# speedinghzl/DSRG

Hardware: AMD Instinct MI355X
Metric: images/sec DSRG train step (VGG16 321x321, 21-class) (higher is better)
Workload: dtype bf16 backbone (fp32 master weights) + f32/f64 supervision path

## Files before the change

dsrg_amd/csrc/conv_direct.hip:

```cpp
#include "common.h"

namespace dsrg {
namespace {
typedef __attribute__((ext_vector_type(8))) __bf16 bf16x8;
typedef __attribute__((ext_vector_type(2))) __bf16 bf16x2;
typedef __attribute__((ext_vector_type(2))) float f32x2;
typedef __attribute__((ext_vector_type(16))) float f32x16;
typedef __attribute__((address_space(3))) void lds_void;
constexpr int kTH = 8, kTW = 16;
constexpr int kHH = kTH + 2, kHW = kTW + 2;

template <int CIN, int COUT, int TPW_ = (CIN == 64 ? 2 : 1)> struct Cfg {
    static constexpr int CG = CIN / 16;
    static constexpr int KS = 9 * CG;
    static constexpr int TPW = TPW_;
    static constexpr int WGS = TPW * KS * 4 <= 144 ? 2 : 1;
    static constexpr int NG = COUT / (32 * TPW);
    static constexpr int PG = 4 / NG;
    static constexpr int MT = 4 / PG;
    static constexpr int KPS = WGS == 2 ? 2 : 4;
    static constexpr int SPT = CG / KPS;
    static constexpr int STEPS = 9 * SPT;
    static constexpr bool DMA = CIN == 128 && COUT == 128;
    static constexpr int CPR = CIN / 8;
    static constexpr int PB = (kHH * kHW + 63) / 64;
    static constexpr int PLANE = PB * 1024;
    static constexpr int NI = CPR * PB;
    static constexpr int IN_STRIDE = CIN * 2 + 16;
    static constexpr int OUT_STRIDE = COUT * 2 + 16;
    static constexpr int IN_BYTES = DMA && CPR * PLANE > kHH * kHW * IN_STRIDE ? CPR * PLANE : kHH * kHW * IN_STRIDE, OUT_BYTES = kTH * kTW * OUT_STRIDE;
    static constexpr int BUF = IN_BYTES > OUT_BYTES ? IN_BYTES : OUT_BYTES;
    static constexpr int VPP = CIN / 8;
    static constexpr int HALO_VECS = kHH * kHW * VPP;
    static constexpr int VPT = (HALO_VECS + 255) / 256;
    static constexpr int VPC = (VPT + MT - 1) / MT;
    static constexpr int OVP = COUT / 8;
    static constexpr int OVT = kTH * kTW * OVP / 256;
    static_assert(NG * PG == 4 && NG >= 1 && MT * PG == 4, "4 waves");
    static_assert(BUF % 16 == 0, "alignment");
};

struct ConvArgs {
    const uint16_t *x;
    const uint16_t *w;
    const float *bias;
    uint16_t *y;
    int B, H, W, relu, tiles_x, tiles_y, ntiles;
    const uint16_t *mask;
    float *colsum;
};

__device__ __forceinline__ uint32_t pack2(float lo, float hi) {
    f32x2 v = {lo, hi};
    bf16x2 b = __builtin_convertvector(v, bf16x2);
    return *reinterpret_cast<uint32_t *>(&b);
}

template <int CIN, int COUT, int TPW_, bool BWD = false>
__global__ __launch_bounds__(256, (TPW_ * CIN <= 64 ? 2 : 1)) void conv3x3_direct_kernel(ConvArgs a) {
    using C = Cfg<CIN, COUT, TPW_>;
    extern __shared__ __attribute__((aligned(16))) unsigned char conv_lds[];
    const int tid = threadIdx.x, lane = tid & 63, wave = tid >> 6;
    const int m = lane & 31, kgrp = lane >> 5;
    const int ng = wave % C::NG, pg = wave / C::NG;

    bf16x8 wf[C::TPW][C::KS];
#pragma unroll
    for (int j = 0; j < C::TPW; j++)
#pragma unroll
        for (int ks = 0; ks < C::KS; ks++)
            wf[j][ks] = *reinterpret_cast<const bf16x8 *>(a.w + (size_t)((ng * C::TPW + j) * 32 + m) * (9 * CIN) + ks * 16 + kgrp * 8);

    constexpr bool kBiasRegs = C::WGS == 1;
    float bias_r[kBiasRegs ? C::TPW : 1][4][4];
    if (kBiasRegs) {
#pragma unroll
        for (int j = 0; j < C::TPW; j++)
#pragma unroll
            for (int q = 0; q < 4; q++)
#pragma unroll
                for (int e = 0; e < 4; e++)
                    bias_r[j][q][e] = a.bias ? a.bias[(ng * C::TPW + j) * 32 + q * 8 + kgrp * 4 + e] : 0.0f;
    }

    auto tile_origin = [&](int t, int &b, int &y0, int &x0) {
        const int per = a.tiles_x * a.tiles_y;
        b = t / per;
        const int r = t - b * per;
        y0 = (r / a.tiles_x) * kTH;
        x0 = (r % a.tiles_x) * kTW;
    };
    constexpr bool kDma = C::DMA && !BWD;
    const rsrc_t rxh = make_rsrc(a.x, (size_t)a.B * a.H * a.W * CIN * 2);
    auto issue_halo = [&](int t, unsigned char *buf) {
        int b, y0, x0;
        tile_origin(t, b, y0, x0);
        const int wv = __builtin_amdgcn_readfirstlane(wave);
        uint32_t poff[C::PB];
#pragma unroll
        for (int blk = 0; blk < C::PB; blk++) {
            const int px = blk * 64 + lane, hy = px / kHW, hx = px - hy * kHW, yy = y0 - 1 + hy, xx = x0 - 1 + hx;
            const bool in = px < kHH * kHW && yy >= 0 && yy < a.H && xx >= 0 && xx < a.W;
            poff[blk] = in ? (uint32_t)((b * a.H + yy) * a.W + xx) * (uint32_t)(CIN * 2) : 0x80000000u;
        }
#pragma unroll
        for (int u = 0; u < (C::NI + 3) / 4; u++) {
            const int q = wv + 4 * u;
            if (q < C::NI) {
                const int c = q / C::PB, blk = q - c * C::PB;
                uint32_t off = poff[0];
#pragma unroll
                for (int k = 1; k < C::PB; k++) off = blk == k ? poff[k] : off;
                __builtin_amdgcn_raw_ptr_buffer_load_lds(rxh, (lds_void *)(buf + q * 1024), 16, off, (uint32_t)(c * 16), 0, 0);
            }
        }
    };
    uint4 pre[C::VPC];
    auto fetch = [&](int t, int c) {
        int b, y0, x0;
        tile_origin(t, b, y0, x0);
#pragma unroll
        for (int u = 0; u < C::VPC; u++) {
            const int v = tid + (c * C::VPC + u) * 256;
            uint4 val = make_uint4(0u, 0u, 0u, 0u);
            if (v < C::HALO_VECS) {
                const int px = v / C::VPP, cg = v % C::VPP, hy = px / kHW, hx = px - hy * kHW;
                const int yy = y0 - 1 + hy, xx = x0 - 1 + hx;
                if (yy >= 0 && yy < a.H && xx >= 0 && xx < a.W)
                    val = *reinterpret_cast<const uint4 *>(a.x + (((size_t)b * a.H + yy) * a.W + xx) * CIN + cg * 8);
            }
            pre[u] = val;
        }
    };
    auto park = [&](unsigned char *buf, int c) {
#pragma unroll
        for (int u = 0; u < C::VPC; u++) {
            const int v = tid + (c * C::VPC + u) * 256;
            if (v < C::HALO_VECS) *reinterpret_cast<uint4 *>(buf + (v / C::VPP) * C::IN_STRIDE + (v % C::VPP) * 16) = pre[u];
        }
    };

    int t = blockIdx.x, cur = 0;
    if (t >= a.ntiles) return;
    if constexpr (kDma) {
        issue_halo(t, conv_lds);
        asm volatile("s_waitcnt vmcnt(0)" ::: "memory");
    } else {
#pragma unroll
        for (int c = 0; c < C::MT; c++) {
            fetch(t, c);
            park(conv_lds, c);
        }
    }
    __syncthreads();
    float *csl = reinterpret_cast<float *>(conv_lds + 2 * C::BUF) + tid * 8;
    if (BWD) {
#pragma unroll
        for (int e = 0; e < 8; e++) csl[e] = 0.0f;
    }
    unsigned char *mtile = conv_lds + 2 * C::BUF + 256 * 8 * sizeof(float);
    const rsrc_t rmask = make_rsrc(a.mask, BWD ? (size_t)a.B * a.H * a.W * COUT * 2 : 0);
    for (; t < a.ntiles; t += gridDim.x) {
        const int tn = t + gridDim.x;
        const bool more = tn < a.ntiles;
        unsigned char *in = conv_lds + cur * C::BUF, *other = conv_lds + (cur ^ 1) * C::BUF;
        if (BWD) {
            int b, y0, x0;
            tile_origin(t, b, y0, x0);
            const int wv = __builtin_amdgcn_readfirstlane(wave);
#pragma unroll
            for (int u = 0; u < C::OVT; u++) {
                const int v = tid + u * 256, px = v / C::OVP, cg = v % C::OVP;
                const int yy = y0 + (px >> 4), xx = x0 + (px & 15);
                const uint32_t off = (yy < a.H && xx < a.W) ? (uint32_t)((b * a.H + yy) * a.W + xx) * (uint32_t)(COUT * 2) + (uint32_t)(cg * 16) : 0x80000000u;
                __builtin_amdgcn_raw_ptr_buffer_load_lds(rmask, (lds_void *)(mtile + (u * 256 + wv * 64) * 16), 16, off, 0, 0, 0);
            }
        }
        if constexpr (kDma)
            if (more) issue_halo(tn, other);
        f32x16 acc[C::MT][C::TPW];
#pragma unroll
        for (int mt = 0; mt < C::MT; mt++) {
            if constexpr (!kDma)
                if (more) fetch(tn, mt);
#pragma unroll
            for (int j = 0; j < C::TPW; j++)
#pragma unroll
                for (int r = 0; r < 16; r++) acc[mt][j][r] = 0.0f;
            const int ty = 2 * (pg * C::MT + mt) + (m >> 4), tx = m & 15;
            const unsigned char *lane_base = kDma ? in + (ty * kHW + tx) * 16 + kgrp * C::PLANE : in + (ty * kHW + tx) * C::IN_STRIDE + kgrp * 16;
            auto a_ptr = [&](int s) {
                const int tap = s / C::SPT, h = s % C::SPT;
                return lane_base + ((tap / 3) * kHW + tap % 3) * (kDma ? 16 : C::IN_STRIDE) + h * (kDma ? 2 * C::KPS * C::PLANE : 32 * C::KPS);
            };
            constexpr int kFragStep = kDma ? 2 * C::PLANE : 32;
            bf16x8 ar[2][C::KPS];
#pragma unroll
            for (int i = 0; i < C::KPS; i++) ar[0][i] = *reinterpret_cast<const bf16x8 *>(a_ptr(0) + i * kFragStep);
#pragma unroll
            for (int s = 0; s < C::STEPS; s++) {
                if (s + 1 < C::STEPS) {
#pragma unroll
                    for (int i = 0; i < C::KPS; i++) ar[(s + 1) & 1][i] = *reinterpret_cast<const bf16x8 *>(a_ptr(s + 1) + i * kFragStep);
                }
                __builtin_amdgcn_sched_barrier(0);
#pragma unroll
                for (int i = 0; i < C::KPS; i++)
#pragma unroll
                    for (int j = 0; j < C::TPW; j++)
                        acc[mt][j] = __builtin_amdgcn_mfma_f32_32x32x16_bf16(wf[j][s * C::KPS + i], ar[s & 1][i], acc[mt][j], 0, 0, 0);
                __builtin_amdgcn_sched_barrier(0);
            }
            if constexpr (!kDma)
                if (more) park(other, mt);
        }
        __syncthreads();
        unsigned char *ot = in;
#pragma unroll
        for (int mt = 0; mt < C::MT; mt++) {
#pragma unroll
            for (int j = 0; j < C::TPW; j++) {
#pragma unroll
                for (int q = 0; q < 4; q++) {
                    const int c0 = (ng * C::TPW + j) * 32 + q * 8 + kgrp * 4;
                    float v[4], bq[4] = {0.0f, 0.0f, 0.0f, 0.0f};
                    if (!kBiasRegs && a.bias) {
                        const float4 b4 = *reinterpret_cast<const float4 *>(a.bias + c0);
                        bq[0] = b4.x; bq[1] = b4.y; bq[2] = b4.z; bq[3] = b4.w;
                    }
#pragma unroll
                    for (int e = 0; e < 4; e++) {
                        v[e] = acc[mt][j][q * 4 + e] + (kBiasRegs ? bias_r[j][q][e] : bq[e]);
                        if (a.relu) v[e] = fmaxf(v[e], 0.0f);
                    }
                    *reinterpret_cast<uint2 *>(ot + ((pg * C::MT + mt) * 32 + m) * C::OUT_STRIDE + c0 * 2) =
                        make_uint2(pack2(v[0], v[1]), pack2(v[2], v[3]));
                }
            }
        }
        if (BWD) asm volatile("s_waitcnt vmcnt(0)" ::: "memory");
        __syncthreads();
        {
            int b, y0, x0;
            tile_origin(t, b, y0, x0);
            float cs[8] = {0.f, 0.f, 0.f, 0.f, 0.f, 0.f, 0.f, 0.f};
#pragma unroll
            for (int u = 0; u < C::OVT; u++) {
                const int v = tid + u * 256, px = v / C::OVP, cg = v % C::OVP;
                const int yy = y0 + (px >> 4), xx = x0 + (px & 15);
                uint4 val = *reinterpret_cast<const uint4 *>(ot + px * C::OUT_STRIDE + cg * 16);
                if (BWD) {
                    uint32_t w4[4] = {val.x, val.y, val.z, val.w};
                    const uint4 mkv = *reinterpret_cast<const uint4 *>(mtile + v * 16);
                    const uint32_t y4[4] = {mkv.x, mkv.y, mkv.z, mkv.w};
#pragma unroll
                    for (int e = 0; e < 4; e++) {
                        w4[e] &= ((int16_t)(y4[e] & 0xffffu) > 0 ? 0x0000ffffu : 0u) | ((int32_t)y4[e] >= 0x10000 ? 0xffff0000u : 0u);
                        cs[2 * e] += __uint_as_float(w4[e] << 16);
                        cs[2 * e + 1] += __uint_as_float(w4[e] & 0xffff0000u);
                    }
                    val = make_uint4(w4[0], w4[1], w4[2], w4[3]);
                }
                if (yy < a.H && xx < a.W)
                    *reinterpret_cast<uint4 *>(a.y + (((size_t)b * a.H + yy) * a.W + xx) * COUT + cg * 8) = val;
            }
            if (BWD) {
#pragma unroll
                for (int e = 0; e < 8; e++) csl[e] += cs[e];
            }
        }
        if constexpr (kDma) asm volatile("s_waitcnt vmcnt(0)" ::: "memory");
        __syncthreads();
        cur ^= 1;
    }
    if (BWD) {
        const float *red = reinterpret_cast<const float *>(conv_lds + 2 * C::BUF);
        __syncthreads();
        if (tid < COUT) {
            const int cg = tid >> 3, e = tid & 7;
            float s0 = 0.0f, s1 = 0.0f;
#pragma unroll 4
            for (int i = 0; i < 256 / C::OVP; i += 2) {
                s0 += red[(cg + C::OVP * i) * 8 + e];
                s1 += red[(cg + C::OVP * (i + 1)) * 8 + e];
            }
            a.colsum[(size_t)blockIdx.x * COUT + tid] = s0 + s1;
        }
    }
}

template <int CIN, int COUT, int TPW_>
int variant_grid(const ConvArgs &a, int n_cus) {
    const int slots = n_cus * Cfg<CIN, COUT, TPW_>::WGS;
    return a.ntiles < slots ? a.ntiles : slots;
}
template <int CIN, int COUT, int TPW_, bool BWD>
int launch_variant(const ConvArgs &a, int n_cus, hipStream_t stream, int &grid) {
    using C = Cfg<CIN, COUT, TPW_>;
    static LdsGrant grant;
    if (C::DMA && !BWD && (size_t)a.B * a.H * a.W * CIN * 2 >= ((size_t)1 << 31)) return DSRG_ERR_UNSUPPORTED;
    grid = variant_grid<CIN, COUT, TPW_>(a, n_cus);
    const size_t lds = 2 * (size_t)C::BUF + (BWD ? 256 * 8 * sizeof(float) + (size_t)kTH * kTW * COUT * 2 : 0);
    if (int rc = ensure_dynamic_lds(reinterpret_cast<const void *>(&conv3x3_direct_kernel<CIN, COUT, TPW_, BWD>), lds, grant)) return rc;
    hipLaunchKernelGGL((conv3x3_direct_kernel<CIN, COUT, TPW_, BWD>), dim3(grid), dim3(256), lds, stream, a);
    DSRG_LAUNCH_CHECK();
    return DSRG_OK;
}
template <int CIN, int COUT, int TPW_>
int launch_shape(const ConvArgs &a, int n_cus, hipStream_t stream, int &grid) {
    return a.mask ? launch_variant<CIN, COUT, TPW_, true>(a, n_cus, stream, grid) : launch_variant<CIN, COUT, TPW_, false>(a, n_cus, stream, grid);
}
constexpr int kC3Pix = 8;

__global__ __launch_bounds__(256) void conv3x3_c3_kernel(ConvArgs a) {
    __shared__ __attribute__((aligned(16))) unsigned char halo[2][kHH * kHW * kC3Pix];
    __shared__ __attribute__((aligned(16))) unsigned char ot[kTH * kTW * 144];
    constexpr int kOutStride = 144;
    const int tid = threadIdx.x, lane = tid & 63, wave = tid >> 6;
    const int m = lane & 31, kgrp = lane >> 5;

    bf16x8 wf[2][3];
#pragma unroll
    for (int nt = 0; nt < 2; nt++)
#pragma unroll
        for (int s3 = 0; s3 < 3; s3++) {
            uint16_t v[8];
#pragma unroll
            for (int e = 0; e < 8; e++) {
                const int tap = 4 * s3 + 2 * kgrp + (e >> 2), c = e & 3;
                v[e] = (tap < 9 && c < 3) ? a.w[((nt * 32 + m) * 9 + tap) * 3 + c] : (uint16_t)0;
            }
            uint4 pk = make_uint4(v[0] | (uint32_t)v[1] << 16, v[2] | (uint32_t)v[3] << 16, v[4] | (uint32_t)v[5] << 16,
                                  v[6] | (uint32_t)v[7] << 16);
            wf[nt][s3] = *reinterpret_cast<bf16x8 *>(&pk);
        }
    float bias_r[2][4][4];
#pragma unroll
    for (int nt = 0; nt < 2; nt++)
#pragma unroll
        for (int q = 0; q < 4; q++)
#pragma unroll
            for (int e = 0; e < 4; e++) bias_r[nt][q][e] = a.bias ? a.bias[nt * 32 + q * 8 + kgrp * 4 + e] : 0.0f;
    int toff[3][2];
#pragma unroll
    for (int s3 = 0; s3 < 3; s3++)
#pragma unroll
        for (int h = 0; h < 2; h++) {
            const int tap = min(4 * s3 + 2 * kgrp + h, 8);
            toff[s3][h] = ((tap / 3) * kHW + tap % 3) * kC3Pix;
        }

    auto tile_origin = [&](int t, int &b, int &y0, int &x0) {
        const int per = a.tiles_x * a.tiles_y;
        b = t / per;
        const int r = t - b * per;
        y0 = (r / a.tiles_x) * kTH;
        x0 = (r % a.tiles_x) * kTW;
    };
    uint2 pre = make_uint2(0u, 0u);
    auto fetch = [&](int t) {
        int b, y0, x0;
        tile_origin(t, b, y0, x0);
        pre = make_uint2(0u, 0u);
        if (tid < kHH * kHW) {
            const int hy = tid / kHW, hx = tid - hy * kHW, yy = y0 - 1 + hy, xx = x0 - 1 + hx;
            if (yy >= 0 && yy < a.H && xx >= 0 && xx < a.W) {
                const uint16_t *p = a.x + (((size_t)b * a.H + yy) * a.W + xx) * 3;
                pre = make_uint2(p[0] | (uint32_t)p[1] << 16, p[2]);
            }
        }
    };
    auto park = [&](unsigned char *buf) {
        if (tid < kHH * kHW) *reinterpret_cast<uint2 *>(buf + tid * kC3Pix) = pre;
    };

    int t = blockIdx.x, cur = 0;
    if (t >= a.ntiles) return;
    fetch(t);
    park(halo[0]);
    __syncthreads();
    const int ty = 2 * wave + (m >> 4), tx = m & 15;
    const int pix_off = (ty * kHW + tx) * kC3Pix;
    for (; t < a.ntiles; t += gridDim.x) {
        const int tn = t + gridDim.x;
        const bool more = tn < a.ntiles;
        if (more) fetch(tn);
        const unsigned char *in = halo[cur] + pix_off;
        f32x16 acc0, acc1;
#pragma unroll
        for (int r = 0; r < 16; r++) { acc0[r] = 0.0f; acc1[r] = 0.0f; }
#pragma unroll
        for (int s3 = 0; s3 < 3; s3++) {
            const uint2 lo = *reinterpret_cast<const uint2 *>(in + toff[s3][0]), hi = *reinterpret_cast<const uint2 *>(in + toff[s3][1]);
            uint4 pk = make_uint4(lo.x, lo.y, hi.x, hi.y);
            const bf16x8 ar = *reinterpret_cast<bf16x8 *>(&pk);
            acc0 = __builtin_amdgcn_mfma_f32_32x32x16_bf16(wf[0][s3], ar, acc0, 0, 0, 0);
            acc1 = __builtin_amdgcn_mfma_f32_32x32x16_bf16(wf[1][s3], ar, acc1, 0, 0, 0);
        }
#pragma unroll
        for (int nt = 0; nt < 2; nt++) {
#pragma unroll
            for (int q = 0; q < 4; q++) {
                const int c0 = nt * 32 + q * 8 + kgrp * 4;
                float v[4];
#pragma unroll
                for (int e = 0; e < 4; e++) {
                    v[e] = (nt ? acc1[q * 4 + e] : acc0[q * 4 + e]) + bias_r[nt][q][e];
                    if (a.relu) v[e] = fmaxf(v[e], 0.0f);
                }
                *reinterpret_cast<uint2 *>(ot + (wave * 32 + m) * kOutStride + c0 * 2) = make_uint2(pack2(v[0], v[1]), pack2(v[2], v[3]));
            }
        }
        if (more) park(halo[cur ^ 1]);
        __syncthreads();
        {
            int b, y0, x0;
            tile_origin(t, b, y0, x0);
#pragma unroll
            for (int u = 0; u < 4; u++) {
                const int v = tid + u * 256, px = v >> 3, cg = v & 7;
                const int yy = y0 + (px >> 4), xx = x0 + (px & 15);
                if (yy < a.H && xx < a.W)
                    *reinterpret_cast<uint4 *>(a.y + (((size_t)b * a.H + yy) * a.W + xx) * 64 + cg * 8) =
                        *reinterpret_cast<const uint4 *>(ot + px * kOutStride + cg * 16);
            }
        }
        __syncthreads();
        cur ^= 1;
    }
}

typedef __attribute__((__vector_size__(4 * sizeof(__bf16)))) __bf16 bf16x4v;
#define DSRG_LDS __attribute__((address_space(3)))

template <int CO_TILES> struct WCfg {
    static constexpr int COUT = 32 * CO_TILES;
    static constexpr int THREADS = CO_TILES * 128;
    static constexpr int NT = 9;
    static constexpr int SX = 192;
    static constexpr int SG = COUT * 2 + 64;
    static constexpr int X_BYTES = kHH * kHW * SX, G_BYTES = kTH * kTW * SG, BUF = X_BYTES + G_BYTES;
    static constexpr int XV = kHH * kHW * 8, XVT = (XV + THREADS - 1) / THREADS;
    static constexpr int GVP = COUT / 8, GVT = kTH * kTW * GVP / THREADS;
    static constexpr int PART = COUT * 9 * 64;
    static constexpr int WGS = CO_TILES == 2 ? 2 : 1, NBUF = WGS == 2 ? 1 : 2;
};

struct WgradArgs {
    const uint16_t *x;
    const uint16_t *g;
    float *part;
    int B, H, W, cin, tiles_x, tiles_y, nitems, roles;
};

__device__ __forceinline__ bf16x8 tr_frag(DSRG_LDS unsigned char *p, int stride4) {
    bf16x4v lo = __builtin_amdgcn_ds_read_tr16_b64_v4bf16(reinterpret_cast<DSRG_LDS bf16x4v *>(p));
    bf16x4v hi = __builtin_amdgcn_ds_read_tr16_b64_v4bf16(reinterpret_cast<DSRG_LDS bf16x4v *>(p + stride4));
    return __builtin_shufflevector(lo, hi, 0, 1, 2, 3, 4, 5, 6, 7);
}

template <int CO_TILES>
__global__ __launch_bounds__(CO_TILES * 128, (CO_TILES == 2 ? 2 : 1)) void conv3x3_wgrad_kernel(WgradArgs a) {
    using C = WCfg<CO_TILES>;
// ... 202 lines not shown
#pragma unroll
    for (int r = 0; r < 16; r++) acc[r] = 0.0f;
    int t = blockIdx.x, cur = 0;
    if (t < a.nitems) {
        fetch(t);
        park(0);
    }
    __syncthreads();
    const int cpx = tid >> 1, chalf = tid & 1;
    const int cty = cpx >> 4, ctx_ = cpx & 15;
    for (; t < a.nitems; t += gridDim.x) {
        const int tn = t + gridDim.x;
        const bool more = tn < a.nitems;
        if (more) fetch(tn);
#pragma unroll
        for (int k = 0; k < 5; k++) {
            const int tap = chalf * 5 + k;
            if (tap < 9)
                *reinterpret_cast<uint2 *>(xc + cpx * kC3Row + tap * 8) =
                    *reinterpret_cast<const uint2 *>(halo(cur) + ((cty + tap / 3) * kHW + ctx_ + tap % 3) * kC3Pix);
        }
        __syncthreads();
        DSRG_LDS unsigned char *gb = (DSRG_LDS unsigned char *)gt(cur) + g_lane, *xb = (DSRG_LDS unsigned char *)xc + x_lane;
#pragma unroll
        for (int ks = 0; ks < kTH; ks++) {
            const bf16x8 ga = tr_frag(gb + ks * kTW * kC3Row, 4 * kC3Row), bx = tr_frag(xb + ks * kTW * kC3Row, 4 * kC3Row);
            acc = __builtin_amdgcn_mfma_f32_32x32x16_bf16(ga, bx, acc, 0, 0, 0);
        }
        if (more) park(cur ^ 1);
        __syncthreads();
        cur ^= 1;
    }
    float *pp = a.part + (size_t)blockIdx.x * 64 * 64;
#pragma unroll
    for (int r = 0; r < 16; r++) {
        const int o = otile * 32 + (r & 3) + 8 * (r >> 2) + 4 * (lane >> 5);
        pp[o * 64 + ntile * 32 + (lane & 31)] = acc[r];
    }
}

template <bool F32_OUT>
__global__ __launch_bounds__(1024) void conv3x3_c3_wgrad_reduce_kernel(const float *part, void *gw, int nwg) {
    __shared__ float red[kRedChunks][64];
    const int el = threadIdx.x & 63, ch = threadIdx.x >> 6;
    const int o = blockIdx.x;
    const float *p = part + o * 64 + el;
    float s = 0.0f;
    for (int w = ch; w < nwg; w += kRedChunks) s += p[(size_t)w * 4096];
    red[ch][el] = s;
    __syncthreads();
    const int tap = el >> 2, c = el & 3;
    if (ch == 0 && tap < 9 && c < 3) {
        float t = 0.0f;
#pragma unroll
        for (int k = 0; k < kRedChunks; k++) t += red[k][el];
        if (F32_OUT) {
            static_cast<float *>(gw)[(o * 9 + tap) * 3 + c] = t;
        } else {
            f32x2 v = {t, 0.0f};
            bf16x2 bv = __builtin_convertvector(v, bf16x2);
            static_cast<uint16_t *>(gw)[(o * 9 + tap) * 3 + c] = *reinterpret_cast<uint16_t *>(&bv);
        }
    }
}

template <int CO_TILES>
int launch_wgrad_variant(const WgradArgs &a, int grid, hipStream_t stream) {
    using C = WCfg<CO_TILES>;
    static LdsGrant grant;
    const size_t lds = C::NBUF * (size_t)C::BUF;
    if (int rc = ensure_dynamic_lds(reinterpret_cast<const void *>(&conv3x3_wgrad_kernel<CO_TILES>), lds, grant)) return rc;
    hipLaunchKernelGGL((conv3x3_wgrad_kernel<CO_TILES>), dim3(grid), dim3(C::THREADS), lds, stream, a);
    DSRG_LAUNCH_CHECK();
    return DSRG_OK;
}

int device_cus() {
    static const int n_cus = [] {
        int dev = 0, n = 0;
        if (hipGetDevice(&dev) != hipSuccess || hipDeviceGetAttribute(&n, hipDeviceAttributeMultiprocessorCount, dev) != hipSuccess || n < 2) n = 256;
        return n;
    }();
    return n_cus;
}

bool wgrad_supported(int cin, int cout) {
    return (cin == 64 && (cout == 64 || cout == 128)) || (cin == 128 && cout == 128) || (cin == 3 && cout == 64);
}

int wgrad_grid(int B, int H, int W, int cin, int cout) {
    const int roles = cin < 64 ? 1 : cin / 64;
    const long items = (long)B * ((W + kTW - 1) / kTW) * ((H + kTH - 1) / kTH) * roles;
    const int per_cu = cout == 64 ? 2 : 1;
    const long cap = (long)device_cus() * per_cu / roles * roles;
    return (int)(items < cap ? items : cap);
}
}

size_t conv3x3_wgrad_workspace(int B, int H, int W, int cin, int cout) {
    if (!wgrad_supported(cin, cout) || B < 1 || H < 1 || W < 1) return 0;
    if (cin == 3) return (size_t)wgrad_grid(B, H, W, cin, cout) * 64 * 64 * sizeof(float);
    return (size_t)wgrad_grid(B, H, W, cin, cout) * cout * 9 * 64 * sizeof(float);
}

int launch_conv3x3_wgrad(const void *x, const void *g, void *gw, float *workspace, size_t workspace_bytes, int B, int H, int W,
                         int cin, int cout, hipStream_t stream, int out_f32) {
    if (!wgrad_supported(cin, cout))
        return set_error(DSRG_ERR_INVALID, "conv3x3_wgrad: %d -> %d channels is not one of 3 -> 64, 64 -> 64, 64 -> 128, 128 -> 128", cin, cout);
    WgradArgs a;
    a.x = static_cast<const uint16_t *>(x); a.g = static_cast<const uint16_t *>(g); a.part = workspace;
    a.B = B; a.H = H; a.W = W; a.cin = cin; a.roles = cin < 64 ? 1 : cin / 64;
    a.tiles_x = (W + kTW - 1) / kTW; a.tiles_y = (H + kTH - 1) / kTH;
    const long items = (long)B * a.tiles_x * a.tiles_y * a.roles;
    if (B < 1 || H < 1 || W < 1 || items > 0x7fffffffL) return set_error(DSRG_ERR_INVALID, "conv3x3_wgrad: bad shape");
    a.nitems = (int)items;
    const int grid = wgrad_grid(B, H, W, cin, cout);
    if (workspace_bytes < conv3x3_wgrad_workspace(B, H, W, cin, cout))
        return set_error(DSRG_ERR_INVALID, "conv3x3_wgrad: workspace of %zu bytes, %zu needed", workspace_bytes,
                         conv3x3_wgrad_workspace(B, H, W, cin, cout));
    if (cin == 3) {
        static LdsGrant grant;
        const size_t lds = 2 * kHH * kHW * kC3Pix + 3 * kTH * kTW * kC3Row;
        if (int rc = ensure_dynamic_lds(reinterpret_cast<const void *>(&conv3x3_c3_wgrad_kernel), lds, grant)) return rc;
        hipLaunchKernelGGL(conv3x3_c3_wgrad_kernel, dim3(grid), dim3(256), lds, stream, a);
        DSRG_LAUNCH_CHECK();
        if (out_f32) hipLaunchKernelGGL(conv3x3_c3_wgrad_reduce_kernel<true>, dim3(64), dim3(1024), 0, stream, workspace, gw, grid);
        else hipLaunchKernelGGL(conv3x3_c3_wgrad_reduce_kernel<false>, dim3(64), dim3(1024), 0, stream, workspace, gw, grid);
        DSRG_LAUNCH_CHECK();
        return DSRG_OK;
    }
    if (int rc = cout == 64 ? launch_wgrad_variant<2>(a, grid, stream) : launch_wgrad_variant<4>(a, grid, stream)) return rc;
    if (out_f32)
        hipLaunchKernelGGL(conv3x3_wgrad_reduce_kernel<true>, dim3(cout * 9 * cin / 64), dim3(1024), 0, stream, workspace, gw, grid, a.roles,
                           cout, cin);
    else
        hipLaunchKernelGGL(conv3x3_wgrad_reduce_kernel<false>, dim3(cout * 9 * cin / 64), dim3(1024), 0, stream, workspace, gw, grid, a.roles,
                           cout, cin);
    DSRG_LAUNCH_CHECK();
    return DSRG_OK;
}

bool conv3x3_direct_supported(int cin, int cout) {
    return ((cin == 64 || cin == 128) && (cout == 64 || cout == 128)) || (cin == 3 && cout == 64);
}

size_t conv3x3_direct_colsum_workspace(int cout) { return (size_t)2 * device_cus() * (size_t)cout * sizeof(float); }

int launch_conv3x3_direct(const void *x, const void *w, const float *bias, void *y, int B, int H, int W, int cin, int cout,
                          int relu, hipStream_t stream, const void *mask, float *colsum, void *colsum_ws, size_t colsum_ws_bytes) {
    if (!conv3x3_direct_supported(cin, cout))
        return set_error(DSRG_ERR_INVALID, "conv3x3_direct: %d -> %d channels is not one of 64/128 -> 64/128 or 3 -> 64", cin, cout);
    if ((mask || colsum) && (cin == 3 || !mask || !colsum))
        return set_error(DSRG_ERR_UNSUPPORTED, "conv3x3_direct: the masked form takes 64 / 128 channels, mask and bias gradient together");
    if (mask && (long long)B * H * W * cout * 2 >= 0x7fffffffLL)
        return set_error(DSRG_ERR_UNSUPPORTED, "conv3x3_direct: mask too large for a 32-bit buffer offset");
    if (colsum && (!colsum_ws || colsum_ws_bytes < conv3x3_direct_colsum_workspace(cout)))
        return set_error(DSRG_ERR_INVALID, "conv3x3_direct: column-sum scratch missing or too small");
    ConvArgs a;
    a.mask = static_cast<const uint16_t *>(mask); a.colsum = colsum ? static_cast<float *>(colsum_ws) : nullptr;
    a.x = static_cast<const uint16_t *>(x); a.w = static_cast<const uint16_t *>(w); a.bias = bias;
    a.y = static_cast<uint16_t *>(y); a.B = B; a.H = H; a.W = W; a.relu = relu ? 1 : 0;
    a.tiles_x = (W + kTW - 1) / kTW; a.tiles_y = (H + kTH - 1) / kTH;
    const long nt = (long)B * a.tiles_x * a.tiles_y;
    if (B < 1 || H < 1 || W < 1 || nt > 0x7fffffffL) return set_error(DSRG_ERR_INVALID, "conv3x3_direct: bad shape");
    a.ntiles = (int)nt;
    const int n_cus = device_cus();
    if (cin == 3) {
        hipLaunchKernelGGL(conv3x3_c3_kernel, dim3(a.ntiles < 4 * n_cus ? a.ntiles : 4 * n_cus), dim3(256), 0, stream, a);
        DSRG_LAUNCH_CHECK();
        return DSRG_OK;
    }
    int rc, grid = 0;
    if (cin == 64 && cout == 64) rc = mask ? launch_variant<64, 64, 2, true>(a, n_cus, stream, grid) : launch_variant<64, 64, 1, false>(a, n_cus, stream, grid);
    else if (cin == 64) rc = launch_shape<64, 128, 2>(a, n_cus, stream, grid);
    else if (cout == 64) rc = launch_shape<128, 64, 1>(a, n_cus, stream, grid);
    else rc = launch_shape<128, 128, 1>(a, n_cus, stream, grid);
    if (rc || !colsum) return rc;
    const float *parts[1] = {a.colsum};
    float *outs[1] = {colsum};
    return launch_igemm_colsum(parts, outs, 1, grid, cout, stream);
}

}
```

Baseline: 1999.

## Rework direct 3x3 conv into multi-buffer DMA ring with per-tile buffer descriptors

Replaces the double-buffered direct conv kernel with an R-deep ring of halo buffers. Every shape, including the backward masked variants, now loads halos through buffer-to-LDS DMA, gated by counted vmcnt waits instead of full drains. Bias moves to LDS, the epilogue uses grouped inline-asm LDS reads and buffer stores, and the tile position is advanced incrementally instead of recomputed with divisions. Per-tile row-based descriptors replace the global 31-bit offset limit. The aim is to overlap global loads with MFMA work across more tiles, at the cost of more LDS per block, fragile hand-written waitcnt accounting, and new per-shape TPW and R choices that may change occupancy.

New measurement: 2018 (median of 6 runs). No clear change (+0.9%).

```diff
diff --git a/dsrg_amd/csrc/conv_direct.hip b/dsrg_amd/csrc/conv_direct.hip
--- a/dsrg_amd/csrc/conv_direct.hip
+++ b/dsrg_amd/csrc/conv_direct.hip
@@ -10,36 +10,6 @@
 constexpr int kTH = 8, kTW = 16;
 constexpr int kHH = kTH + 2, kHW = kTW + 2;
 
-template <int CIN, int COUT, int TPW_ = (CIN == 64 ? 2 : 1)> struct Cfg {
-    static constexpr int CG = CIN / 16;
-    static constexpr int KS = 9 * CG;
-    static constexpr int TPW = TPW_;
-    static constexpr int WGS = TPW * KS * 4 <= 144 ? 2 : 1;
-    static constexpr int NG = COUT / (32 * TPW);
-    static constexpr int PG = 4 / NG;
-    static constexpr int MT = 4 / PG;
-    static constexpr int KPS = WGS == 2 ? 2 : 4;
-    static constexpr int SPT = CG / KPS;
-    static constexpr int STEPS = 9 * SPT;
-    static constexpr bool DMA = CIN == 128 && COUT == 128;
-    static constexpr int CPR = CIN / 8;
-    static constexpr int PB = (kHH * kHW + 63) / 64;
-    static constexpr int PLANE = PB * 1024;
-    static constexpr int NI = CPR * PB;
-    static constexpr int IN_STRIDE = CIN * 2 + 16;
-    static constexpr int OUT_STRIDE = COUT * 2 + 16;
-    static constexpr int IN_BYTES = DMA && CPR * PLANE > kHH * kHW * IN_STRIDE ? CPR * PLANE : kHH * kHW * IN_STRIDE, OUT_BYTES = kTH * kTW * OUT_STRIDE;
-    static constexpr int BUF = IN_BYTES > OUT_BYTES ? IN_BYTES : OUT_BYTES;
-    static constexpr int VPP = CIN / 8;
-    static constexpr int HALO_VECS = kHH * kHW * VPP;
-    static constexpr int VPT = (HALO_VECS + 255) / 256;
-    static constexpr int VPC = (VPT + MT - 1) / MT;
-    static constexpr int OVP = COUT / 8;
-    static constexpr int OVT = kTH * kTW * OVP / 256;
-    static_assert(NG * PG == 4 && NG >= 1 && MT * PG == 4, "4 waves");
-    static_assert(BUF % 16 == 0, "alignment");
-};
-
 struct ConvArgs {
     const uint16_t *x;
     const uint16_t *w;
@@ -56,13 +26,99 @@
     return *reinterpret_cast<uint32_t *>(&b);
 }
 
-template <int CIN, int COUT, int TPW_, bool BWD = false>
-__global__ __launch_bounds__(256, (TPW_ * CIN <= 64 ? 2 : 1)) void conv3x3_direct_kernel(ConvArgs a) {
-    using C = Cfg<CIN, COUT, TPW_>;
+template <int CIN, int COUT, int TPW_, bool BWD, int R_> struct Cfg {
+    static constexpr int CG = CIN / 16;
+    static constexpr int KS = 9 * CG;
+    static constexpr int TPW = TPW_;
+    static constexpr int NG = COUT / (32 * TPW);
+    static constexpr int PG = 4 / NG;
+    static constexpr int MT = 4 / PG;
+    static constexpr int R = R_;
+    static constexpr int CPR = CIN / 8;
+    static constexpr int PB = (kHH * kHW + 63) / 64;
+    static constexpr int PLANE = PB * 1024;
+    static constexpr int NI = CPR * PB;
+    static constexpr int HALO = CPR * PLANE;
+    static constexpr int OUT_STRIDE = COUT * 2 + 16;
+    static constexpr int OUT_BYTES = kTH * kTW * OUT_STRIDE;
+    static constexpr bool SEP = OUT_BYTES > HALO;
+    static constexpr int OVP = COUT / 8;
+    static constexpr int OVT = kTH * kTW * OVP / 256;
+    static constexpr int HI = NI / 4, ST = OVT, MK = BWD ? OVT : 0;
+    static constexpr int WAIT_NEXT = (R - 1) * ST + (R - 2) * (MK + HI);
+    static constexpr int OFF_OT = R * HALO;
+    static constexpr int OFF_BIAS = OFF_OT + (SEP ? OUT_BYTES : 0);
+    static constexpr int OFF_CS = OFF_BIAS + COUT * 4;
+    static constexpr int OFF_MASK = OFF_CS + (BWD ? 256 * 8 * 4 : 0);
+    static constexpr int LDS = OFF_MASK + (BWD ? kTH * kTW * COUT * 2 : 0);
+    static constexpr int WGS = (TPW * KS * 4 <= 144 && 2 * LDS <= 160 * 1024) ? 2 : 1;
+    static constexpr int KPS = WGS == 2 ? 2 : 4;
+    static constexpr int SPT = CG / KPS;
+    static constexpr int STEPS = 9 * SPT;
+    static constexpr int SG = (BWD && CIN == 128 && COUT == 128) ? 2 : 4;
+    static_assert(NG * PG == 4 && NG >= 1 && MT * PG == 4, "4 waves");
+    static_assert(NI % 4 == 0 && R >= 2 && WAIT_NEXT <= 63 && HI <= 63, "the vmcnt field");
+    static_assert(HALO % 16 == 0 && OUT_BYTES % 16 == 0 && LDS <= 160 * 1024, "LDS");
+};
+
+constexpr uint32_t kOutOfRange = 0x80000000u;
+inline bool ring_rows_addressable(int W, int cin, int cout) {
+    return (unsigned long long)kHH * (unsigned long long)W * (unsigned long long)(cin > cout ? cin : cout) * 2ull < (unsigned long long)kOutOfRange;
+}
+struct TilePos { int b, ty, tx; };
+
+__device__ __forceinline__ int fresh(int v) {
+    asm volatile("" : "+v"(v));
+    return v;
+}
+__device__ __forceinline__ uint32_t lds_addr(const void *p) {
+    return (uint32_t)(uintptr_t)(const __attribute__((address_space(3))) void *)p;
+}
+__device__ __forceinline__ void lds_write_b64(uint32_t addr, int off, uint32_t lo, uint32_t hi) {
+    const uint64_t d = (uint64_t)hi << 32 | lo;
+    asm volatile("ds_write_b64 %0, %1 offset:%2" ::"v"(addr), "v"(d), "n"(off));
+}
+template <typename V = decltype(__builtin_amdgcn_raw_buffer_load_b128(rsrc_t(), 0, 0, 0))>
+__device__ __forceinline__ V lds_read_b128(uint32_t addr, int off) {
+    V d;
+    asm volatile("ds_read_b128 %0, %1 offset:%2\n\ts_waitcnt lgkmcnt(0)" : "=v"(d) : "v"(addr), "n"(off));
+    return d;
+}
+template <int N, int STEP, int STEP2, bool TWO, typename V>
+__device__ __forceinline__ void lds_read_group(uint32_t addr, uint32_t addr2, V (&d)[N], V (&e)[N]) {
+    static_assert(N == 2 || N == 4, "group size");
+    if constexpr (N == 2 && !TWO)
+        asm volatile("ds_read_b128 %0, %2\n\tds_read_b128 %1, %2 offset:%3\n\ts_waitcnt lgkmcnt(0)"
+                     : "=&v"(d[0]), "=&v"(d[1]) : "v"(addr), "n"(STEP));
+    else if constexpr (N == 2)
+        asm volatile("ds_read_b128 %0, %4\n\tds_read_b128 %1, %4 offset:%6\n\tds_read_b128 %2, %5\n\tds_read_b128 %3, %5 offset:%7\n\t"
+                     "s_waitcnt lgkmcnt(0)"
+                     : "=&v"(d[0]), "=&v"(d[1]), "=&v"(e[0]), "=&v"(e[1]) : "v"(addr), "v"(addr2), "n"(STEP), "n"(STEP2));
+    else if constexpr (!TWO)
+        asm volatile("ds_read_b128 %0, %4\n\tds_read_b128 %1, %4 offset:%5\n\tds_read_b128 %2, %4 offset:%6\n\tds_read_b128 %3, %4 offset:%7\n\t"
+                     "s_waitcnt lgkmcnt(0)"
+                     : "=&v"(d[0]), "=&v"(d[1]), "=&v"(d[2]), "=&v"(d[3]) : "v"(addr), "n"(STEP), "n"(2 * STEP), "n"(3 * STEP));
+    else
+        asm volatile("ds_read_b128 %0, %8\n\tds_read_b128 %1, %8 offset:%10\n\tds_read_b128 %2, %8 offset:%11\n\tds_read_b128 %3, %8 offset:%12\n\t"
+                     "ds_read_b128 %4, %9\n\tds_read_b128 %5, %9 offset:%13\n\tds_read_b128 %6, %9 offset:%14\n\tds_read_b128 %7, %9 offset:%15\n\t"
+                     "s_waitcnt lgkmcnt(0)"
+                     : "=&v"(d[0]), "=&v"(d[1]), "=&v"(d[2]), "=&v"(d[3]), "=&v"(e[0]), "=&v"(e[1]), "=&v"(e[2]), "=&v"(e[3])
+                     : "v"(addr), "v"(addr2), "n"(STEP), "n"(2 * STEP), "n"(3 * STEP), "n"(STEP2), "n"(2 * STEP2), "n"(3 * STEP2));
+}
+template <int N> __device__ __forceinline__ void vm_wait() { asm volatile("s_waitcnt vmcnt(%0)" ::"n"(N) : "memory"); }
+template <int N> __device__ __forceinline__ void vm_wait_barrier() { asm volatile("s_waitcnt vmcnt(%0) lgkmcnt(0)\n\ts_barrier" ::"n"(N) : "memory"); }
+__device__ __forceinline__ void lds_barrier() { asm volatile("s_waitcnt lgkmcnt(0)\n\ts_barrier" ::: "memory"); }
+
+template <int CIN, int COUT, int TPW_, bool BWD, int R_>
+__global__ __launch_bounds__(256, (Cfg<CIN, COUT, TPW_, BWD, R_>::WGS)) void conv3x3_direct_kernel(ConvArgs a) {
+    using C = Cfg<CIN, COUT, TPW_, BWD, R_>;
+    using u32x4 = decltype(__builtin_amdgcn_raw_buffer_load_b128(rsrc_t(), 0, 0, 0));
     extern __shared__ __attribute__((aligned(16))) unsigned char conv_lds[];
     const int tid = threadIdx.x, lane = tid & 63, wave = tid >> 6;
     const int m = lane & 31, kgrp = lane >> 5;
     const int ng = wave % C::NG, pg = wave / C::NG;
+    const int wv = __builtin_amdgcn_readfirstlane(wave);
+    if ((int)blockIdx.x >= a.ntiles) return;
 
     bf16x8 wf[C::TPW][C::KS];
 #pragma unroll
@@ -71,129 +127,99 @@
         for (int ks = 0; ks < C::KS; ks++)
             wf[j][ks] = *reinterpret_cast<const bf16x8 *>(a.w + (size_t)((ng * C::TPW + j) * 32 + m) * (9 * CIN) + ks * 16 + kgrp * 8);
 
-    constexpr bool kBiasRegs = C::WGS == 1;
-    float bias_r[kBiasRegs ? C::TPW : 1][4][4];
-    if (kBiasRegs) {
-#pragma unroll
-        for (int j = 0; j < C::TPW; j++)
-#pragma unroll
-            for (int q = 0; q < 4; q++)
-#pragma unroll
-                for (int e = 0; e < 4; e++)
-                    bias_r[j][q][e] = a.bias ? a.bias[(ng * C::TPW + j) * 32 + q * 8 + kgrp * 4 + e] : 0.0f;
-    }
-
-    auto tile_origin = [&](int t, int &b, int &y0, int &x0) {
-        const int per = a.tiles_x * a.tiles_y;
-        b = t / per;
-        const int r = t - b * per;
-        y0 = (r / a.tiles_x) * kTH;
-        x0 = (r % a.tiles_x) * kTW;
-    };
-    constexpr bool kDma = C::DMA && !BWD;
-    const rsrc_t rxh = make_rsrc(a.x, (size_t)a.B * a.H * a.W * CIN * 2);
-    auto issue_halo = [&](int t, unsigned char *buf) {
-        int b, y0, x0;
-        tile_origin(t, b, y0, x0);
-        const int wv = __builtin_amdgcn_readfirstlane(wave);
+    float *biasl = reinterpret_cast<float *>(conv_lds + C::OFF_BIAS);
+    if (tid < COUT) biasl[tid] = a.bias ? a.bias[tid] : 0.0f;
+    float *csl = reinterpret_cast<float *>(conv_lds + C::OFF_CS) + tid * 8;
+    if (BWD) {
+#pragma unroll
+        for (int e = 0; e < 8; e++) csl[e] = 0.0f;
+    }
+    unsigned char *mtile = conv_lds + C::OFF_MASK;
+    __builtin_amdgcn_s_waitcnt(0x0f70);
+
+    const int per = a.tiles_x * a.tiles_y;
+    TilePos pos[C::R];
+    {
+        const int t0 = blockIdx.x;
+        pos[0].b = t0 / per;
+        const int r = t0 - pos[0].b * per;
+        pos[0].ty = r / a.tiles_x;
+        pos[0].tx = r - pos[0].ty * a.tiles_x;
+    }
+    const int step_b = (int)gridDim.x / per, step_r = (int)gridDim.x - step_b * per;
+    const int step_y = step_r / a.tiles_x, step_x = step_r - step_y * a.tiles_x;
+    auto advance = [&](const TilePos &p) {
+        TilePos q;
+        q.tx = p.tx + step_x;
+        const int cx = q.tx >= a.tiles_x ? 1 : 0;
+        q.tx -= cx * a.tiles_x;
+        q.ty = p.ty + step_y + cx;
+        const int cy = q.ty >= a.tiles_y ? 1 : 0;
+        q.ty -= cy * a.tiles_y;
+        q.b = p.b + step_b + cy;
+        return q;
+    };
+#pragma unroll
+    for (int k = 1; k < C::R; k++) pos[k] = advance(pos[k - 1]);
+
+    auto issue_halo = [&](const TilePos &p, unsigned char *buf) {
+        const int y0 = p.ty * kTH, x0 = p.tx * kTW;
+        const bool live = p.b < a.B;
+        const rsrc_t rx = make_rsrc(a.x + ((long long)p.b * a.H + (y0 - 1)) * (long long)a.W * CIN, (size_t)kHH * a.W * CIN * 2);
         uint32_t poff[C::PB];
+        const int ln = fresh(lane);
 #pragma unroll
         for (int blk = 0; blk < C::PB; blk++) {
-            const int px = blk * 64 + lane, hy = px / kHW, hx = px - hy * kHW, yy = y0 - 1 + hy, xx = x0 - 1 + hx;
-            const bool in = px < kHH * kHW && yy >= 0 && yy < a.H && xx >= 0 && xx < a.W;
-            poff[blk] = in ? (uint32_t)((b * a.H + yy) * a.W + xx) * (uint32_t)(CIN * 2) : 0x80000000u;
-        }
-#pragma unroll
-        for (int u = 0; u < (C::NI + 3) / 4; u++) {
+            const int px = blk * 64 + ln, hy = px / kHW, hx = px - hy * kHW, yy = y0 - 1 + hy, xx = x0 - 1 + hx;
+            const bool in = live & (px < kHH * kHW) & (yy >= 0) & (yy < a.H) & (xx >= 0) & (xx < a.W);
+            poff[blk] = in ? (uint32_t)(hy * a.W + xx) * (uint32_t)(CIN * 2) : kOutOfRange;
+        }
+#pragma unroll
+        for (int u = 0; u < C::HI; u++) {
             const int q = wv + 4 * u;
-            if (q < C::NI) {
-                const int c = q / C::PB, blk = q - c * C::PB;
-                uint32_t off = poff[0];
-#pragma unroll
-                for (int k = 1; k < C::PB; k++) off = blk == k ? poff[k] : off;
-                __builtin_amdgcn_raw_ptr_buffer_load_lds(rxh, (lds_void *)(buf + q * 1024), 16, off, (uint32_t)(c * 16), 0, 0);
-            }
-        }
-    };
-    uint4 pre[C::VPC];
-    auto fetch = [&](int t, int c) {
-        int b, y0, x0;
-        tile_origin(t, b, y0, x0);
-#pragma unroll
-        for (int u = 0; u < C::VPC; u++) {
-            const int v = tid + (c * C::VPC + u) * 256;
-            uint4 val = make_uint4(0u, 0u, 0u, 0u);
-            if (v < C::HALO_VECS) {
-                const int px = v / C::VPP, cg = v % C::VPP, hy = px / kHW, hx = px - hy * kHW;
-                const int yy = y0 - 1 + hy, xx = x0 - 1 + hx;
-                if (yy >= 0 && yy < a.H && xx >= 0 && xx < a.W)
-                    val = *reinterpret_cast<const uint4 *>(a.x + (((size_t)b * a.H + yy) * a.W + xx) * CIN + cg * 8);
-            }
-            pre[u] = val;
-        }
-    };
-    auto park = [&](unsigned char *buf, int c) {
-#pragma unroll
-        for (int u = 0; u < C::VPC; u++) {
-            const int v = tid + (c * C::VPC + u) * 256;
-            if (v < C::HALO_VECS) *reinterpret_cast<uint4 *>(buf + (v / C::VPP) * C::IN_STRIDE + (v % C::VPP) * 16) = pre[u];
-        }
-    };
-
-    int t = blockIdx.x, cur = 0;
-    if (t >= a.ntiles) return;
-    if constexpr (kDma) {
-        issue_halo(t, conv_lds);
-        asm volatile("s_waitcnt vmcnt(0)" ::: "memory");
-    } else {
-#pragma unroll
-        for (int c = 0; c < C::MT; c++) {
-            fetch(t, c);
-            park(conv_lds, c);
-        }
-    }
-    __syncthreads();
-    float *csl = reinterpret_cast<float *>(conv_lds + 2 * C::BUF) + tid * 8;
-    if (BWD) {
-#pragma unroll
-        for (int e = 0; e < 8; e++) csl[e] = 0.0f;
-    }
-    unsigned char *mtile = conv_lds + 2 * C::BUF + 256 * 8 * sizeof(float);
-    const rsrc_t rmask = make_rsrc(a.mask, BWD ? (size_t)a.B * a.H * a.W * COUT * 2 : 0);
-    for (; t < a.ntiles; t += gridDim.x) {
-        const int tn = t + gridDim.x;
-        const bool more = tn < a.ntiles;
-        unsigned char *in = conv_lds + cur * C::BUF, *other = conv_lds + (cur ^ 1) * C::BUF;
-        if (BWD) {
-            int b, y0, x0;
-            tile_origin(t, b, y0, x0);
-            const int wv = __builtin_amdgcn_readfirstlane(wave);
-#pragma unroll
-            for (int u = 0; u < C::OVT; u++) {
-                const int v = tid + u * 256, px = v / C::OVP, cg = v % C::OVP;
-                const int yy = y0 + (px >> 4), xx = x0 + (px & 15);
-                const uint32_t off = (yy < a.H && xx < a.W) ? (uint32_t)((b * a.H + yy) * a.W + xx) * (uint32_t)(COUT * 2) + (uint32_t)(cg * 16) : 0x80000000u;
-                __builtin_amdgcn_raw_ptr_buffer_load_lds(rmask, (lds_void *)(mtile + (u * 256 + wv * 64) * 16), 16, off, 0, 0, 0);
-            }
-        }
-        if constexpr (kDma)
-            if (more) issue_halo(tn, other);
+            const int c = q / C::PB, blk = q - c * C::PB;
+            uint32_t off = poff[0];
+#pragma unroll
+            for (int k = 1; k < C::PB; k++) off = blk == k ? poff[k] : off;
+            __builtin_amdgcn_raw_ptr_buffer_load_lds(rx, (lds_void *)(buf + q * 1024), 16, off, (uint32_t)(c * 16), 0, 0);
+        }
+    };
+    auto out_off = [&](int td, int u, int y0, int x0) {
+        const int v = td + u * 256, px = v / C::OVP, cg = v % C::OVP;
+        const int r = px >> 4, xx = x0 + (px & 15);
+        return ((y0 + r < a.H) & (xx < a.W)) ? (uint32_t)(r * a.W + xx) * (uint32_t)(COUT * 2) + (uint32_t)(cg * 16) : kOutOfRange;
+    };
+
+    auto issue_mask = [&](long long row0, int y0, int x0) {
+        const rsrc_t rmask = make_rsrc(a.mask + row0, (size_t)kTH * a.W * COUT * 2);
+        const int td = fresh(tid);
+#pragma unroll
+        for (int u = 0; u < C::OVT; u++) {
+            const uint32_t off = out_off(td, u, y0, x0);
+            __builtin_amdgcn_raw_ptr_buffer_load_lds(rmask, (lds_void *)(mtile + (u * 256 + wv * 64) * 16), 16, off, 0, 0, 0);
+        }
+    };
+
+    int cur = 0;
+#pragma unroll
+    for (int k = 0; k + 1 < C::R; k++) issue_halo(pos[k], conv_lds + k * C::HALO);
+    vm_wait_barrier<0>();
+    for (;;) {
+        unsigned char *in = conv_lds + cur * C::HALO;
+        const int y0 = pos[0].ty * kTH, x0 = pos[0].tx * kTW;
+        const long long row0 = ((long long)pos[0].b * a.H + y0) * (long long)a.W * COUT;
+        if (BWD) issue_mask(row0, y0, x0);
+        issue_halo(pos[C::R - 1], conv_lds + (cur == 0 ? C::R - 1 : cur - 1) * C::HALO);
         f32x16 acc[C::MT][C::TPW];
 #pragma unroll
         for (int mt = 0; mt < C::MT; mt++) {
-            if constexpr (!kDma)
-                if (more) fetch(tn, mt);
-#pragma unroll
-            for (int j = 0; j < C::TPW; j++)
-#pragma unroll
-                for (int r = 0; r < 16; r++) acc[mt][j][r] = 0.0f;
             const int ty = 2 * (pg * C::MT + mt) + (m >> 4), tx = m & 15;
-            const unsigned char *lane_base = kDma ? in + (ty * kHW + tx) * 16 + kgrp * C::PLANE : in + (ty * kHW + tx) * C::IN_STRIDE + kgrp * 16;
+            const unsigned char *lane_base = in + (ty * kHW + tx) * 16 + kgrp * C::PLANE;
             auto a_ptr = [&](int s) {
                 const int tap = s / C::SPT, h = s % C::SPT;
-                return lane_base + ((tap / 3) * kHW + tap % 3) * (kDma ? 16 : C::IN_STRIDE) + h * (kDma ? 2 * C::KPS * C::PLANE : 32 * C::KPS);
+                return lane_base + ((tap / 3) * kHW + tap % 3) * 16 + h * (2 * C::KPS * C::PLANE);
             };
-            constexpr int kFragStep = kDma ? 2 * C::PLANE : 32;
+            constexpr int kFragStep = 2 * C::PLANE;
             bf16x8 ar[2][C::KPS];
 #pragma unroll
             for (int i = 0; i < C::KPS; i++) ar[0][i] = *reinterpret_cast<const bf16x8 *>(a_ptr(0) + i * kFragStep);
@@ -208,73 +234,84 @@
                 for (int i = 0; i < C::KPS; i++)
 #pragma unroll
                     for (int j = 0; j < C::TPW; j++)
-                        acc[mt][j] = __builtin_amdgcn_mfma_f32_32x32x16_bf16(wf[j][s * C::KPS + i], ar[s & 1][i], acc[mt][j], 0, 0, 0);
+                        acc[mt][j] = __builtin_amdgcn_mfma_f32_32x32x16_bf16(wf[j][s * C::KPS + i], ar[s & 1][i], s + i == 0 ? f32x16{} : acc[mt][j], 0, 0, 0);
                 __builtin_amdgcn_sched_barrier(0);
             }
-            if constexpr (!kDma)
-                if (more) park(other, mt);
-        }
-        __syncthreads();
-        unsigned char *ot = in;
+        }
+        if (!C::SEP) lds_barrier();
+        unsigned char *ot = C::SEP ? conv_lds + C::OFF_OT : in;
+        const uint32_t bias_lane = lds_addr(biasl + ng * C::TPW * 32 + kgrp * 4);
+        u32x4 bv[C::TPW][4];
+#pragma unroll
+        for (int j = 0; j < C::TPW; j++) lds_read_group<4, 32, 0, false>(bias_lane + j * 128, 0u, bv[j], bv[j]);
+        const uint32_t ot_lane = lds_addr(ot + (pg * C::MT * 32 + m) * C::OUT_STRIDE + (ng * C::TPW * 32 + kgrp * 4) * 2);
 #pragma unroll
         for (int mt = 0; mt < C::MT; mt++) {
 #pragma unroll
             for (int j = 0; j < C::TPW; j++) {
 #pragma unroll
                 for (int q = 0; q < 4; q++) {
-                    const int c0 = (ng * C::TPW + j) * 32 + q * 8 + kgrp * 4;
-                    float v[4], bq[4] = {0.0f, 0.0f, 0.0f, 0.0f};
-                    if (!kBiasRegs && a.bias) {
-                        const float4 b4 = *reinterpret_cast<const float4 *>(a.bias + c0);
-                        bq[0] = b4.x; bq[1] = b4.y; bq[2] = b4.z; bq[3] = b4.w;
-                    }
+                    const u32x4 b4 = bv[j][q];
+                    const float bq[4] = {__uint_as_float(b4[0]), __uint_as_float(b4[1]), __uint_as_float(b4[2]), __uint_as_float(b4[3])};
+                    float v[4];
 #pragma unroll
                     for (int e = 0; e < 4; e++) {
-                        v[e] = acc[mt][j][q * 4 + e] + (kBiasRegs ? bias_r[j][q][e] : bq[e]);
+                        v[e] = acc[mt][j][q * 4 + e] + bq[e];
                         if (a.relu) v[e] = fmaxf(v[e], 0.0f);
                     }
-                    *reinterpret_cast<uint2 *>(ot + ((pg * C::MT + mt) * 32 + m) * C::OUT_STRIDE + c0 * 2) =
-                        make_uint2(pack2(v[0], v[1]), pack2(v[2], v[3]));
+                    lds_write_b64(ot_lane, (mt * 32) * C::OUT_STRIDE + (j * 32 + q * 8) * 2, pack2(v[0], v[1]), pack2(v[2], v[3]));
                 }
             }
         }
-        if (BWD) asm volatile("s_waitcnt vmcnt(0)" ::: "memory");
-        __syncthreads();
+        if (BWD) vm_wait<C::HI>();
+        lds_barrier();
         {
-            int b, y0, x0;
-            tile_origin(t, b, y0, x0);
+            const rsrc_t ry = make_rsrc(a.y + row0, (size_t)kTH * a.W * COUT * 2);
             float cs[8] = {0.f, 0.f, 0.f, 0.f, 0.f, 0.f, 0.f, 0.f};
-#pragma unroll
-            for (int u = 0; u < C::OVT; u++) {
-                const int v = tid + u * 256, px = v / C::OVP, cg = v % C::OVP;
-                const int yy = y0 + (px >> 4), xx = x0 + (px & 15);
-                uint4 val = *reinterpret_cast<const uint4 *>(ot + px * C::OUT_STRIDE + cg * 16);
-                if (BWD) {
-                    uint32_t w4[4] = {val.x, val.y, val.z, val.w};
-                    const uint4 mkv = *reinterpret_cast<const uint4 *>(mtile + v * 16);
-                    const uint32_t y4[4] = {mkv.x, mkv.y, mkv.z, mkv.w};
-#pragma unroll
-                    for (int e = 0; e < 4; e++) {
-                        w4[e] &= ((int16_t)(y4[e] & 0xffffu) > 0 ? 0x0000ffffu : 0u) | ((int32_t)y4[e] >= 0x10000 ? 0xffff0000u : 0u);
-                        cs[2 * e] += __uint_as_float(w4[e] << 16);
-                        cs[2 * e + 1] += __uint_as_float(w4[e] & 0xffff0000u);
+            const int td = fresh(tid);
+            const uint32_t ot_rd = lds_addr(ot + (td / C::OVP) * C::OUT_STRIDE + (td % C::OVP) * 16), mk_rd = lds_addr(mtile + td * 16);
+#pragma unroll C::SG == 2 ? 1 : C::OVT / C::SG
+            for (int u0 = 0; u0 < C::OVT; u0 += C::SG) {
+                u32x4 ov[C::SG], mk[C::SG];
+                constexpr int kOtStep = (256 / C::OVP) * C::OUT_STRIDE;
+                lds_read_group<C::SG, kOtStep, 4096, BWD>(ot_rd + u0 * kOtStep, mk_rd + u0 * 4096, ov, mk);
+#pragma unroll
+                for (int k = 0; k < C::SG; k++) {
+                    u32x4 sv = ov[k];
+                    if (BWD) {
+#pragma unroll
+                        for (int e = 0; e < 4; e++) {
+                            const uint32_t y = mk[k][e];
+                            sv[e] &= ((int16_t)(y & 0xffffu) > 0 ? 0x0000ffffu : 0u) | ((int32_t)y >= 0x10000 ? 0xffff0000u : 0u);
+                            cs[2 * e] += __uint_as_float(sv[e] << 16);
+                            cs[2 * e + 1] += __uint_as_float(sv[e] & 0xffff0000u);
+                        }
                     }
-                    val = make_uint4(w4[0], w4[1], w4[2], w4[3]);
+                    __builtin_amdgcn_raw_buffer_store_b128(sv, ry, out_off(td, u0 + k, y0, x0), 0, 0);
                 }
-                if (yy < a.H && xx < a.W)
-                    *reinterpret_cast<uint4 *>(a.y + (((size_t)b * a.H + yy) * a.W + xx) * COUT + cg * 8) = val;
             }
             if (BWD) {
-#pragma unroll
-                for (int e = 0; e < 8; e++) csl[e] += cs[e];
-            }
-        }
-        if constexpr (kDma) asm volatile("s_waitcnt vmcnt(0)" ::: "memory");
-        __syncthreads();
-        cur ^= 1;
-    }
+                const uint32_t cs_lane = lds_addr(csl);
+                const u32x4 s0 = lds_read_b128(cs_lane, 0), s1 = lds_read_b128(cs_lane, 16);
+#pragma unroll
+                for (int e = 0; e < 4; e++) {
+                    cs[e] += __uint_as_float(s0[e]);
+                    cs[4 + e] += __uint_as_float(s1[e]);
+                }
+#pragma unroll
+                for (int e = 0; e < 8; e += 2) lds_write_b64(cs_lane, e * 4, __float_as_uint(cs[e]), __float_as_uint(cs[e + 1]));
+            }
+        }
+#pragma unroll
+        for (int k = 0; k + 1 < C::R; k++) pos[k] = pos[k + 1];
+        pos[C::R - 1] = advance(pos[C::R - 1]);
+        cur = cur == C::R - 1 ? 0 : cur + 1;
+        vm_wait_barrier<C::WAIT_NEXT>();
+        if (pos[0].b >= a.B) break;
+    }
+    vm_wait<0>();
     if (BWD) {
-        const float *red = reinterpret_cast<const float *>(conv_lds + 2 * C::BUF);
+        const float *red = reinterpret_cast<const float *>(conv_lds + C::OFF_CS);
         __syncthreads();
         if (tid < COUT) {
             const int cg = tid >> 3, e = tid & 7;
@@ -289,26 +326,15 @@
     }
 }
 
-template <int CIN, int COUT, int TPW_>
-int variant_grid(const ConvArgs &a, int n_cus) {
-    const int slots = n_cus * Cfg<CIN, COUT, TPW_>::WGS;
-    return a.ntiles < slots ? a.ntiles : slots;
-}
-template <int CIN, int COUT, int TPW_, bool BWD>
-int launch_variant(const ConvArgs &a, int n_cus, hipStream_t stream, int &grid) {
-    using C = Cfg<CIN, COUT, TPW_>;
+template <int CIN, int COUT, int TPW_, bool BWD, int R_>
+int launch_ring(const ConvArgs &a, int n_cus, hipStream_t stream, int &grid) {
+    using C = Cfg<CIN, COUT, TPW_, BWD, R_>;
     static LdsGrant grant;
-    if (C::DMA && !BWD && (size_t)a.B * a.H * a.W * CIN * 2 >= ((size_t)1 << 31)) return DSRG_ERR_UNSUPPORTED;
-    grid = variant_grid<CIN, COUT, TPW_>(a, n_cus);
-    const size_t lds = 2 * (size_t)C::BUF + (BWD ? 256 * 8 * sizeof(float) + (size_t)kTH * kTW * COUT * 2 : 0);
-    if (int rc = ensure_dynamic_lds(reinterpret_cast<const void *>(&conv3x3_direct_kernel<CIN, COUT, TPW_, BWD>), lds, grant)) return rc;
-    hipLaunchKernelGGL((conv3x3_direct_kernel<CIN, COUT, TPW_, BWD>), dim3(grid), dim3(256), lds, stream, a);
+    grid = a.ntiles < n_cus * C::WGS ? a.ntiles : n_cus * C::WGS;
+    if (int rc = ensure_dynamic_lds(reinterpret_cast<const void *>(&conv3x3_direct_kernel<CIN, COUT, TPW_, BWD, R_>), C::LDS, grant)) return rc;
+    hipLaunchKernelGGL((conv3x3_direct_kernel<CIN, COUT, TPW_, BWD, R_>), dim3(grid), dim3(256), C::LDS, stream, a);
     DSRG_LAUNCH_CHECK();
     return DSRG_OK;
-}
-template <int CIN, int COUT, int TPW_>
-int launch_shape(const ConvArgs &a, int n_cus, hipStream_t stream, int &grid) {
-    return a.mask ? launch_variant<CIN, COUT, TPW_, true>(a, n_cus, stream, grid) : launch_variant<CIN, COUT, TPW_, false>(a, n_cus, stream, grid);
 }
 constexpr int kC3Pix = 8;
 
@@ -817,8 +843,6 @@
         return set_error(DSRG_ERR_INVALID, "conv3x3_direct: %d -> %d channels is not one of 64/128 -> 64/128 or 3 -> 64", cin, cout);
     if ((mask || colsum) && (cin == 3 || !mask || !colsum))
         return set_error(DSRG_ERR_UNSUPPORTED, "conv3x3_direct: the masked form takes 64 / 128 channels, mask and bias gradient together");
-    if (mask && (long long)B * H * W * cout * 2 >= 0x7fffffffLL)
-        return set_error(DSRG_ERR_UNSUPPORTED, "conv3x3_direct: mask too large for a 32-bit buffer offset");
     if (colsum && (!colsum_ws || colsum_ws_bytes < conv3x3_direct_colsum_workspace(cout)))
         return set_error(DSRG_ERR_INVALID, "conv3x3_direct: column-sum scratch missing or too small");
     ConvArgs a;
@@ -835,11 +859,13 @@
         DSRG_LAUNCH_CHECK();
         return DSRG_OK;
     }
+    if (!ring_rows_addressable(W, cin, cout))
+        return set_error(DSRG_ERR_UNSUPPORTED, "conv3x3_direct: ten rows of %d pixels exceed a 31-bit buffer offset", W);
     int rc, grid = 0;
-    if (cin == 64 && cout == 64) rc = mask ? launch_variant<64, 64, 2, true>(a, n_cus, stream, grid) : launch_variant<64, 64, 1, false>(a, n_cus, stream, grid);
-    else if (cin == 64) rc = launch_shape<64, 128, 2>(a, n_cus, stream, grid);
-    else if (cout == 64) rc = launch_shape<128, 64, 1>(a, n_cus, stream, grid);
-    else rc = launch_shape<128, 128, 1>(a, n_cus, stream, grid);
+    if (cin == 64 && cout == 64) rc = mask ? launch_ring<64, 64, 1, true, 2>(a, n_cus, stream, grid) : launch_ring<64, 64, 1, false, 2>(a, n_cus, stream, grid);
+    else if (cin == 64) rc = mask ? launch_ring<64, 128, 1, true, 3>(a, n_cus, stream, grid) : launch_ring<64, 128, 2, false, 2>(a, n_cus, stream, grid);
+    else if (cout == 64) rc = mask ? launch_ring<128, 64, 1, true, 2>(a, n_cus, stream, grid) : launch_ring<128, 64, 1, false, 2>(a, n_cus, stream, grid);
+    else rc = mask ? launch_ring<128, 128, 1, true, 2>(a, n_cus, stream, grid) : launch_ring<128, 128, 1, false, 2>(a, n_cus, stream, grid);
     if (rc || !colsum) return rc;
     const float *parts[1] = {a.colsum};
     float *outs[1] = {colsum};
```
